# bassamlab/SigmaRL

Measured on AMD Instinct MI355X. Metric: env-steps/sec (agents x envs x steps), CPM scenario, 16 agents (open loop, 32 steps per launch), higher is better.
Workload: dtype f32

## Files before the change

sigmarl_amd/csrc/sigmaenv.hip:

```cpp
#include <hip/hip_runtime.h>

#include <algorithm>
#include <atomic>
#include <cmath>
#include <cstdio>
#include <cstdlib>
#include <cstring>
#include <string>
#include <type_traits>
#include <vector>

#include "sigmaenv_device.h"

using namespace sigmadev;

#ifdef SIGMAENV_PROFILE
#define PROF_TS2(g, tid, k) do { if ((g).dbg_ts2 && (tid) == 0) (g).dbg_ts2[(size_t)blockIdx.x * 16 + (k)] = __builtin_readcyclecounter(); } while (0)
#else
#define PROF_TS2(g, tid, k) do { } while (0)
#endif

#include "../../include/sigmaenv_ref_weights.h"
static_assert(NS >= 1 && NS <= SIGMAENV_MAX_SHORT_TERM, "SIGMAENV_N_SHORT_TERM out of range");
__device__ __constant__ uint32_t W_REF_BITS[NS] = SIGMAENV_W_REF_BITS;

#define AUTO_RESET_MAX_TRIES 64

#define DIST_STRIDE(N) ((N) + 1)
#define COL_STRIDE(N) ((N) + 4)
#define ESCR_BYTES (8 * 4 * 4 * 16)
#define CAND_LIST 16
#define ITEM_CAP(S) ((S) * 24 > 64 ? (S) * 24 : 64)
#define NEAR_CAP 8
struct Smem {
  float *st, *vold, *vnew, *shrt, *dref, *dleft, *dright, *dbound, *dist, *obs, *thr, *cs, *rew;
  float* carry;
  int *path, *cp, *near, *flags, *npts;
  unsigned long long* cmask;
  uint8_t* cand;
  uint16_t* pidx;
  float4* escr;
  uint8_t* col;
  uint16_t* items;
  unsigned long long* acc64;
  uint32_t* acc32;
  int* nearn;
  uint8_t* nearl;
  uint8_t* fresh;
  unsigned long long* key64;
  __host__ __device__ static __forceinline__ size_t scan_scratch_ints(int S) {
    return (size_t)S * 3 * 2 + (size_t)S * 2 * 4 + (size_t)S * 2 + (size_t)(ITEM_CAP(S) + 1) / 2 + (size_t)(S * 2 * NEAR_CAP + 3) / 4;
  }
  __host__ __device__ static __forceinline__ size_t stage_floats(int S, int D, bool lean) {
    const size_t o = ((size_t)S * D + 3) & ~(size_t)3, q = (scan_scratch_ints(S) + 3) & ~(size_t)3;
    return (lean && q > o) ? q : o;
  }
  __device__ __forceinline__ Smem(char* base, int S, int N, int K, int D, bool lean = false) {
    escr = reinterpret_cast<float4*>(base);
    float* f = reinterpret_cast<float*>(base + (lean ? 0 : ESCR_BYTES));
    obs = f;
    {
      int* q = reinterpret_cast<int*>(f);
      acc64 = reinterpret_cast<unsigned long long*>(q); q += S * 3 * 2;
      acc32 = reinterpret_cast<uint32_t*>(q); q += S * 2 * 4;
      nearn = q; q += S * 2;
      items = reinterpret_cast<uint16_t*>(q); q += (ITEM_CAP(S) + 1) / 2;
      nearl = reinterpret_cast<uint8_t*>(q);
    }
    f += stage_floats(S, D, lean);
    st = f; f += S * 8;
    vold = f; f += S * 10;
    vnew = f; f += S * 10;
    shrt = f; f += S * NS * 2;
    dref = f; f += S;
    dleft = f; f += S * 5;
    dright = f; f += S * 5;
    dbound = f; f += S;
    dist = f; f += S * DIST_STRIDE(N);
    thr = f; f += S * 3;
    cs = f; f += S * 2;
    rew = f; f += S * 2;
    carry = f; f += S * 3;
    int* i = reinterpret_cast<int*>(f);
    path = i; i += S;
    cp = i; i += S * 3;
    near = i; i += S * (K > 0 ? K : 1);
    flags = i; i += S * 4;
    npts = i; i += S * 3;
    i += ((reinterpret_cast<uintptr_t>(i) >> 2) & 1);
    cmask = reinterpret_cast<unsigned long long*>(i);
    if (!lean) i += S * 3 * 2;
    key64 = lean ? reinterpret_cast<unsigned long long*>(i) : cmask;
    if (lean) i += S * 2;
    cand = reinterpret_cast<uint8_t*>(i);
    if (!lean) i += S * 3 * (CAND_LIST / 4);
    pidx = reinterpret_cast<uint16_t*>(i); i += (N * (N - 1) / 2 + 1) / 2;
    col = reinterpret_cast<uint8_t*>(i);
    fresh = col + (size_t)S * COL_STRIDE(N);
  }
  __host__ __device__ static __forceinline__ size_t bytes(int S, int N, int K, int D, bool lean = false) {
    size_t f = stage_floats(S, D, lean) + (size_t)S * 8 + S * 10 * 2 + S * NS * 2 + S + S * 5 * 2 + S + (size_t)S * DIST_STRIDE(N) + S * 3 + S * 2 + S * 2 + S * 3;
    size_t i = (size_t)S + S * 3 + S * (K > 0 ? K : 1) + S * 4 + S * 3 + 1;
    i += lean ? (size_t)S * 2 : ((size_t)S * 3 * 2 + (size_t)S * 3 * (CAND_LIST / 4));
    return (lean ? 0 : ESCR_BYTES) + (f + i + (size_t)(N * (N - 1) / 2 + 1) / 2) * 4 + (size_t)S * COL_STRIDE(N) + (((size_t)S + 3) & ~(size_t)3) + 16;
  }
};

__device__ __forceinline__ void wave_sync() {
  __builtin_amdgcn_fence(__ATOMIC_RELEASE, "wavefront");
  __builtin_amdgcn_wave_barrier();
  __builtin_amdgcn_fence(__ATOMIC_ACQUIRE, "wavefront");
}
template <bool WAVE>
struct Grp {
  __device__ static __forceinline__ int tid() {
    if (!WAVE) return (int)threadIdx.x;
    int x = (int)(threadIdx.x & 63);
    asm volatile("" : "+v"(x));
    __builtin_assume(x >= 0 && x < 64);
    return x;
  }
  __device__ static __forceinline__ int size() { return WAVE ? 64 : (int)blockDim.x; }
  __device__ static __forceinline__ void sync() { if (WAVE) wave_sync(); else __syncthreads(); }
};

struct ObsLayout {
  int F, bird, full, p_steer, p_short, p_dcen, p_bnd, n_bnd_pts, own_w, oth_w, q_vel, q_steer, q_dist, q_ref, n_oth_pts, T1, pad, D, DL;
  int W_oth;
  enum { F_VERT, F_POS, F_ROT, F_LEN, F_WID, F_VEL, F_STEER, F_DIST, F_REF };
  __host__ __device__ __forceinline__ bool feature(int idx, int N, int& kind, int& wid) const {
    int n = 0;
#define SIGMA_FEAT(cond, k_, w_) if (cond) { if (idx == n) { kind = (k_); wid = (w_); return true; } ++n; }
    const bool nv = (F & SIGMAENV_OBS_NO_VERTICES) != 0;
    SIGMA_FEAT(!nv, F_VERT, 8)
    SIGMA_FEAT(nv, F_POS, 2) SIGMA_FEAT(nv, F_ROT, 1) SIGMA_FEAT(nv, F_LEN, 1) SIGMA_FEAT(nv, F_WID, 1)
    SIGMA_FEAT(true, F_VEL, 2)
    SIGMA_FEAT((F & SIGMAENV_OBS_STEERING) != 0, F_STEER, 1)
    SIGMA_FEAT(!(F & SIGMAENV_OBS_NO_DIST_AGENTS), F_DIST, N)
    SIGMA_FEAT((F & SIGMAENV_OBS_REF_OTHERS) != 0, F_REF, 2 * NS)
#undef SIGMA_FEAT
    return false;
  }
  __host__ __device__ __forceinline__ ObsLayout(int F_, int N, int K) {
    F = F_;
    bird = (F & SIGMAENV_OBS_BIRD_VIEW) != 0;
    full = (F & SIGMAENV_OBS_FULL) != 0;
    int p = bird ? 5 : 1;
    p_steer = (F & SIGMAENV_OBS_STEERING) ? p++ : -1;
    p_short = p; p += 2 * NS;
    p_dcen = (F & SIGMAENV_OBS_NO_DIST_CENTER) ? -1 : p++;
// ... 2248 lines not shown
```

sigmarl_amd/csrc/sigmaenv_step_wave.inc:

```

__device__ __forceinline__ float dpp_swap1(float v) {
  return __int_as_float(__builtin_amdgcn_update_dpp(0, __float_as_int(v), 0xB1, 0xF, 0xF, true));
}

__device__ __forceinline__ void bicycle_step_pair(const sigmaenv_config_t& c, const CfgDerived& dv, float s[8], float u0, float u1, float uc[2], float cs_yaw[2], bool par, int h, float cr[3]) {
  const float a0 = clampf(u0, -c.max_speed, c.max_speed);
  const float a1 = clampf(u1, -c.max_steering, c.max_steering);
  uc[0] = a0;
  uc[1] = a1;
  float x = s[0], y = s[1], psi = s[2], v = s[3], delta = s[4];
  float u_acc = (a0 - v) / c.dt;
  float u_sr = (a1 - delta) / c.dt;
  u_acc = clampf(u_acc, c.min_acc, c.max_acc);
  u_sr = clampf(u_sr, c.min_steering_rate, c.max_steering_rate);
  const float l_wb = dv.l_wb, k_beta = dv.k_beta;
  const float dt = c.dt;
  float delta_new = delta + dt * u_sr;
  delta_new = remainder_pos(delta_new + PI32, TWO_PI32) - PI32;
  float tan_d, beta, beta1, tan_new;
  {
    const float x1 = (par && h) ? delta_new : delta;
    const float t1 = cr_tan(x1);
    const float b1 = cr_atan(k_beta * t1);
    if (par) {
// ... 49 lines not shown
      c1 = ca;
      cr_sincos(psi, sy, cy);
    }
  }
  s[0] = x; s[1] = y; s[2] = psi; s[3] = v; s[4] = delta_new;
  s[5] = v * c1;
  s[6] = v * s1;
  s[7] = beta1;
  cs_yaw[0] = cy;
  cs_yaw[1] = sy;
  cr[0] = tan_new; cr[1] = c1; cr[2] = s1;
}

__device__ __forceinline__ void bicycle_step_pair_carried(const sigmaenv_config_t& c, const CfgDerived& dv, float s[8], float u0, float u1, float uc[2], float cs_yaw[2], int h, float cr[3]) {
  const float a0 = clampf(u0, -c.max_speed, c.max_speed);
  const float a1 = clampf(u1, -c.max_steering, c.max_steering);
  uc[0] = a0;
  uc[1] = a1;
  float x = s[0], y = s[1], psi = s[2], v = s[3], delta = s[4];
  const float beta = s[7];
  float u_acc = (a0 - v) / c.dt;
  float u_sr = (a1 - delta) / c.dt;
  u_acc = clampf(u_acc, c.min_acc, c.max_acc);
  u_sr = clampf(u_sr, c.min_steering_rate, c.max_steering_rate);
  const float l_wb = dv.l_wb, k_beta = dv.k_beta;
  const float dt = c.dt;
  float delta_new = delta + dt * u_sr;
  delta_new = remainder_pos(delta_new + PI32, TWO_PI32) - PI32;
  double sd, cd;
  sigma_sincos_f64((double)(h ? delta_new : beta), &sd, &cd);
  const float t1 = (float)(sd / cd);
  const float b1 = cr_atan(k_beta * t1);
  const float cb = (float)cd;
  const float t1o = dpp_swap1(t1), b1o = dpp_swap1(b1), cbo = dpp_swap1(cb);
  const float tan_new = h ? t1 : t1o, beta1 = h ? b1 : b1o, cosb = h ? cbo : cb;
  const float tan_d = cr[0], c0 = cr[1], s0 = cr[2];
  const float dx0 = v * c0;
  const float dx1 = v * s0;
  const float dx2 = (v / l_wb) * tan_d * cosb;
  x = x + dt * dx0;
  y = y + dt * dx1;
  psi = psi + dt * dx2;
  v = v + dt * u_acc;
  const float course = psi + beta1;
  float sa, ca;
  cr_sincos(h ? psi : course, sa, ca);
  const float so = dpp_swap1(sa), co = dpp_swap1(ca);
  const float s1 = h ? so : sa, c1 = h ? co : ca, sy = h ? sa : so, cy = h ? ca : co;
  s[0] = x; s[1] = y; s[2] = psi; s[3] = v; s[4] = delta_new;
  s[5] = v * c1;
  s[6] = v * s1;
  s[7] = beta1;
  cs_yaw[0] = cy;
  cs_yaw[1] = sy;
  cr[0] = tan_new; cr[1] = c1; cr[2] = s1;
}

__device__ __forceinline__ void rect_vertices_cs(const CfgDerived& dv, float px, float py, float cs, float sn, float* v ) {
  const float lh = dv.lh, wh = dv.wh;
  const float nsn = -sn;
  const float bx[5] = {lh, lh, -lh, -lh, lh};
  const float by[5] = {wh, -wh, -wh, wh, wh};
#pragma unroll
  for (int k = 0; k < 5; ++k) {
    v[2 * k] = (cs * bx[k] + nsn * by[k]) + px;
    v[2 * k + 1] = (sn * bx[k] + cs * by[k]) + py;
  }
}

__device__ __forceinline__ int wave_inclusive_sum(int v, int ) {
  v += __builtin_amdgcn_update_dpp(0, v, 0x111, 0xF, 0xF, false);
  v += __builtin_amdgcn_update_dpp(0, v, 0x112, 0xF, 0xF, false);
  v += __builtin_amdgcn_update_dpp(0, v, 0x114, 0xF, 0xF, false);
  v += __builtin_amdgcn_update_dpp(0, v, 0x118, 0xF, 0xF, false);
  v += __builtin_amdgcn_update_dpp(0, v, 0x142, 0xA, 0xF, false);
  v += __builtin_amdgcn_update_dpp(0, v, 0x143, 0xC, 0xF, false);
  return v;
}

struct ScanItemOut {
  float best;
  int bk;
  float bs0, bs1, bs2, bs3;
};

template <bool FASTDIV, int SEGS>
__device__ __forceinline__ void scan_chunk(const DevMap& m, const Smem& s, int sl, int pl, unsigned poly_off, int npt, int ch, int u0, bool first_of_env,
                                           const float near_thr, ScanItemOut& o) {
  const float cgx = s.st[sl * 8], cgy = s.st[sl * 8 + 1];
  const unsigned kmax = (unsigned)(npt - 2 < 0 ? 0 : npt - 2);
  Seg4 sg[SEGS];
#pragma unroll
  for (int u = 0; u < SEGS; ++u) {
    const unsigned k = min((unsigned)(ch * SIGMAENV_CHUNK + u0 + u), kmax);
    sg[u] = *reinterpret_cast<const Seg4*>(m.center + (poly_off + 2u * k));
  }
  const float* qv = first_of_env ? (s.vold + sl * 10) : (s.vnew + sl * 10);
  float q0x = 0.f, q0y = 0.f, q1x = 0.f, q1y = 0.f, q2x = 0.f, q2y = 0.f, q3x = 0.f, q3y = 0.f;
  if (pl != 0) { q0x = qv[0]; q0y = qv[1]; q1x = qv[2]; q1y = qv[3]; q2x = qv[4]; q2y = qv[5]; q3x = qv[6]; q3y = qv[7]; }
  o.bs0 = INFINITY; o.bs1 = INFINITY; o.bs2 = INFINITY; o.bs3 = INFINITY;
  unsigned near_bits = 0u;
  const float near_thr_up = __uint_as_float(__float_as_uint(near_thr) + 1u);
  float zc[SEGS];
  float zbest = INFINITY;
#pragma unroll
  for (int u = 0; u < SEGS; ++u) {
    const int k = ch * SIGMAENV_CHUNK + u0 + u;
    const bool valid = k + 1 < npt;
    const float ax = sg[u].ax, ay = sg[u].ay;
    const float lx = sg[u].bx - ax, ly = sg[u].by - ay;
    const float len2 = lx * lx + ly * ly;
    const float rcp = FASTDIV ? shared_rcp(len2) : 0.0f;
    const float z0 = point_segment_sq_t<FASTDIV>(cgx, cgy, ax, ay, lx, ly, len2, rcp);
    zc[u] = z0;
    if (valid && z0 < zbest) zbest = z0;
    if (pl != 0) {
      const float v0 = point_segment_sq_t<FASTDIV>(q0x, q0y, ax, ay, lx, ly, len2, rcp);
      const float v1 = point_segment_sq_t<FASTDIV>(q1x, q1y, ax, ay, lx, ly, len2, rcp);
      const float v2 = point_segment_sq_t<FASTDIV>(q2x, q2y, ax, ay, lx, ly, len2, rcp);
      const float v3 = point_segment_sq_t<FASTDIV>(q3x, q3y, ax, ay, lx, ly, len2, rcp);
      if (valid) {
        o.bs0 = fmin_nc(o.bs0, v0); o.bs1 = fmin_nc(o.bs1, v1); o.bs2 = fmin_nc(o.bs2, v2); o.bs3 = fmin_nc(o.bs3, v3);
        if (!(fmaf(-near_thr_up, near_thr, z0) > 0.0f)) near_bits |= 1u << u;
      }
    }
  }
  {
    const float d = sqrtf(zbest);
    const float d_up = __uint_as_float(__float_as_uint(d) + 1u);
    o.best = d; o.bk = 0x7FFFFFFF;
#pragma unroll
    for (int u = SEGS - 1; u >= 0; --u) {
      const int k = ch * SIGMAENV_CHUNK + u0 + u;
      if (k + 1 < npt && fmaf(-d_up, d, zc[u]) <= 0.0f) o.bk = k;
    }
  }
  if (near_bits) {
    const int bt = sl * 2 + (pl - 1);
    int slot = atomicAdd(&s.nearn[bt], (int)__popc(near_bits));
#pragma unroll
    for (int u = 0; u < SEGS; ++u) {
      if ((near_bits >> u) & 1u) {
        if (slot < NEAR_CAP) s.nearl[bt * NEAR_CAP + slot] = (uint8_t)(ch * SIGMAENV_CHUNK + u0 + u);
        ++slot;
      }
    }
  }
}
__device__ __forceinline__ void scan_merge(const Smem& s, int sl, int pl, const ScanItemOut& o) {
  if (o.bk != 0x7FFFFFFF) {
    const unsigned long long key = ((unsigned long long)__float_as_uint(o.best) << 32) | (unsigned)o.bk;
    atomicMin(&s.acc64[sl * 3 + pl], key);
  }
  if (pl != 0) {
    uint32_t* a = s.acc32 + (sl * 2 + (pl - 1)) * 4;
    atomicMin(&a[0], __float_as_uint(o.bs0)); atomicMin(&a[1], __float_as_uint(o.bs1));
    atomicMin(&a[2], __float_as_uint(o.bs2)); atomicMin(&a[3], __float_as_uint(o.bs3));
  }
}

template <bool FASTDIV>
__device__ __forceinline__ void scan_tile_balanced(const DevMap& m, const CfgDerived& dv, const DevBufs& g, const Smem& s, const Tile& t, int G, int lane) {
  const int N = t.N, slots = t.slots, SG = G * N, n_tasks = SG * 3, cap = ITEM_CAP(SG);
  const float near_thr = m.rect_radius + 1e-4f;
  for (int base = 0; base < n_tasks; base += 64) {
    const int tl = base + lane;
    const int grp_raw = fdiv(tl, g.mSG), sl_raw = tl - grp_raw * SG;
    const int pl_raw = grp_raw >= 2 ? 0 : grp_raw + 1;
    const int tpm = pl_raw * SG + sl_raw;
    const bool act = tl < n_tasks && sl_raw < slots;
    const int pl = act ? pl_raw : 0, sl = act ? sl_raw : 0;
    const int task = sl * 3 + pl;
    unsigned long long mk = 0ull;
#ifdef SIGMAENV_PROFILE
    int lvl_prof = 0;
#endif
    if (act) {
      MaskTask mt;
      mask_stage1(m, mt, task, s.path[sl], s.cp[task]);
      mask_stage2<true>(m, s, mt, true, N);
#ifdef SIGMAENV_PROFILE
      lvl_prof = mt.lvl;
#endif
      const float px = mt.px, py = mt.py, T2 = mt.T2;
      const int nch = mt.nch;
      unsigned long long rest = mt.rest;
      if (mt.fast && mt.own < nch) { mk |= 1ull << mt.own; rest &= ~(1ull << mt.own); }
      while (rest) {
        int idx[8];
#pragma unroll
        for (int q = 0; q < 8; ++q) { idx[q] = rest ? (__ffsll((long long)rest) - 1) : -1; rest &= rest - 1ull; }
        float4 b[8];
#pragma unroll
        for (int q = 0; q < 8; ++q) b[q] = mt.box[idx[q] < 0 ? 0 : idx[q]];
#pragma unroll
        for (int q = 0; q < 8; ++q) {
          if (idx[q] >= 0 && idx[q] < nch && box_within(b[q], px, py, T2)) mk |= 1ull << idx[q];
        }
      }
      if (!mt.fast) {
        const float4* gbox = m.group_box + ((size_t)mt.path * 3 + pl) * 8;
        unsigned gm = 0u;
#pragma unroll 1
        for (int gidx = 0; gidx < 8; ++gidx) {
          if (gidx * 8 < nch && box_within(gbox[gidx], px, py, T2)) gm |= 1u << gidx;
        }
        while (gm) {
          const int gidx = __ffs((int)gm) - 1;
          gm &= gm - 1u;
#pragma unroll 1
          for (int q = 0; q < 8; ++q) {
            const int cidx = gidx * 8 + q;
            if (cidx < nch && box_within(mt.box[cidx], px, py, T2)) mk |= 1ull << cidx;
          }
        }
      }
      s.npts[task] = mt.npt;
      s.acc64[task] = ~0ull;
      if (pl != 0) {
        const int bt = sl * 2 + (pl - 1);
        uint32_t* a = s.acc32 + bt * 4;
        a[0] = 0x7F800000u; a[1] = 0x7F800000u; a[2] = 0x7F800000u; a[3] = 0x7F800000u;
        s.nearn[bt] = 0;
      }
    }
#ifdef SIGMAENV_PROFILE
    if (g.dbg_ts && lane == 0 && base == 0) g.dbg_ts[(size_t)t.env0 / (size_t)G * 16 + 10] = __builtin_readcyclecounter();
    {
      const unsigned long long bfar = __ballot(act && lvl_prof >= 2), btight = __ballot(act && lvl_prof == 0);
#ifndef SIGMAENV_PROFILE_RT
      if (g.dbg_ts && lane == 0) {
        unsigned long long* row = g.dbg_ts + (size_t)t.env0 / (size_t)G * 16;
        row[12] += (unsigned long long)__popcll(bfar); row[13] += bfar ? 1ull : 0ull; row[14] += (unsigned long long)__popcll(btight);
        row[15] += (unsigned long long)__popcll(bfar & 0x0000000100010001ull);
      }
#endif
    }
#endif
    bool pending = act;
    do {
      const int cnt = pending ? __popcll(mk) : 0;
      const int incl = wave_inclusive_sum(cnt, lane);
      const int off = incl - cnt;
      const bool listed = pending && off + cnt <= cap;
      if (listed) {
        int j = off;
        while (mk) {
          const int ch = __ffsll((long long)mk) - 1;
          mk &= mk - 1ull;
          s.items[j++] = (uint16_t)((tpm << 6) | ch);
        }
      }
      const unsigned long long unl = __ballot(pending && !listed);
      const int total = unl ? __builtin_amdgcn_readlane(off, __builtin_amdgcn_readfirstlane(__ffsll((long long)unl) - 1)) : __builtin_amdgcn_readlane(incl, 63);
      pending = pending && !listed;
      wave_sync();
#ifdef SIGMAENV_PROFILE
      if (g.dbg_ts && lane == 0) {
        g.dbg_ts[(size_t)t.env0 / (size_t)G * 16 + 8] += (unsigned long long)total;
        g.dbg_ts[(size_t)t.env0 / (size_t)G * 16 + 9] += 1ull;
      }
#endif
      auto item_part = [&](int it, auto segs_tag, int u0) {
        constexpr int SEGS = decltype(segs_tag)::value;
        const unsigned code = s.items[it];
        const int tpm2 = (int)(code >> 6), ch = (int)(code & 63u);
        const int pl2 = fdiv(tpm2, g.mSG), sl2 = tpm2 - pl2 * SG;
        const bool first = (sl2 - fdiv(sl2, g.mN) * N) == 0;
        ScanItemOut o;
        const unsigned poly_off = (unsigned)pl2 * (unsigned)m.poly_stride + (unsigned)s.path[sl2] * (unsigned)(m.P * 2);
        scan_chunk<FASTDIV, SEGS>(m, s, sl2, pl2, poly_off, s.npts[sl2 * 3 + pl2], ch, u0, first, near_thr, o);
        scan_merge(s, sl2, pl2, o);
      };
      int it0 = 0;
      for (; it0 + 64 <= total; it0 += 64) item_part(it0 + lane, std::integral_constant<int, SIGMAENV_CHUNK>{}, 0);
      const int rem = total - it0;
      if (rem > 32) {
        if (lane < rem) item_part(it0 + lane, std::integral_constant<int, SIGMAENV_CHUNK>{}, 0);
      } else if (rem > 16) {
        if ((lane >> 1) < rem) item_part(it0 + (lane >> 1), std::integral_constant<int, SIGMAENV_CHUNK / 2>{}, (lane & 1) * (SIGMAENV_CHUNK / 2));
      } else if (rem > 0) {
        if ((lane >> 2) < rem) item_part(it0 + (lane >> 2), std::integral_constant<int, SIGMAENV_CHUNK / 4>{}, (lane & 3) * (SIGMAENV_CHUNK / 4));
      }
      wave_sync();
    } while (__any(pending));
  }
#ifdef SIGMAENV_PROFILE
  if (g.dbg_ts && lane == 0) g.dbg_ts[(size_t)t.env0 / (size_t)G * 16 + 11] = __builtin_readcyclecounter();
#endif
  const float wh = dv.wh;
  for (int tpm = lane; tpm < n_tasks; tpm += 64) {
    const int pl = fdiv(tpm, g.mSG), sl = tpm - pl * SG;
    if (sl >= slots) continue;
    const unsigned long long key = s.acc64[sl * 3 + pl];
    const float best = __uint_as_float((uint32_t)(key >> 32));
    const int bk = (int)(uint32_t)key;
    s.cp[sl * 3 + pl] = bk + 1;
    if (pl == 0) {
      s.dref[sl] = best;
    } else {
      float* dst = (pl == 1 ? s.dleft : s.dright) + sl * 5;
      dst[0] = best - wh;
    }
  }
  for (int w = lane; w < slots * 8; w += 64) {
    const int bt = w >> 2, q = w & 3, sl = bt >> 1;
    float* dst = ((bt & 1) ? s.dright : s.dleft) + sl * 5;
    dst[1 + q] = sqrtf(__uint_as_float(s.acc32[w]));
  }
}

template <int SN>
struct PairTable {
  uint16_t v[SN * (SN - 1) / 2 > 0 ? SN * (SN - 1) / 2 : 1];
  constexpr PairTable() : v() {
    int k = 0;
    for (int i = 0; i < SN - 1; ++i)
      for (int j = i + 1; j < SN; ++j) v[k++] = (uint16_t)(i | (j << 8));
  }
};
template <int SN>
__device__ const PairTable<SN> kPairTable{};

#ifndef STEP_WAVE_MIN_WAVES
#define STEP_WAVE_MIN_WAVES 4
#endif
struct StepKernArgs {
  DevMap m;
  DevBufs g;
  const float* actions_base;
  float* slab_base;
  size_t act_stride, slab_stride;
  uint64_t seed, counter0;
  int G_arg, tile_lds, path_first, path_count, n_steps;
};
template <class T>
__device__ __forceinline__ T* as_global(T* p) {
  return (T*)(__attribute__((address_space(1))) T*)p;
}
#define SIGMA_COPY_GLOBAL(dst, src, f) dst.f = as_global(src.f)
__device__ __forceinline__ void load_step_tables(const __attribute__((address_space(4))) StepKernArgs* ka, DevMap& m, DevBufs& g) {
  SIGMA_COPY_GLOBAL(m, ka->m, center); SIGMA_COPY_GLOBAL(m, ka->m, left); SIGMA_COPY_GLOBAL(m, ka->m, right); SIGMA_COPY_GLOBAL(m, ka->m, yaw);
  SIGMA_COPY_GLOBAL(m, ka->m, n_center); SIGMA_COPY_GLOBAL(m, ka->m, n_left); SIGMA_COPY_GLOBAL(m, ka->m, n_right); SIGMA_COPY_GLOBAL(m, ka->m, is_loop);
  SIGMA_COPY_GLOBAL(m, ka->m, chunk_box); SIGMA_COPY_GLOBAL(m, ka->m, group_box); SIGMA_COPY_GLOBAL(m, ka->m, chunk_neigh); SIGMA_COPY_GLOBAL(m, ka->m, start_table);
  m.P = ka->m.P; m.n_paths = ka->m.n_paths; m.yaw_stride = ka->m.yaw_stride; m.neigh_radius = ka->m.neigh_radius; m.neigh_radius_far = ka->m.neigh_radius_far;
  m.nch = ka->m.nch; m.fast_div = ka->m.fast_div; m.rect_radius = ka->m.rect_radius; m.poly_stride = ka->m.poly_stride;
  m.n_lists = ka->m.n_lists; m.neigh_radius_tight = ka->m.neigh_radius_tight;
  m.list_first16 = ka->m.list_first16; m.list_count16 = ka->m.list_count16; m.cdf0 = ka->m.cdf0; m.cdf1 = ka->m.cdf1; m.cdf2 = ka->m.cdf2;
  SIGMA_COPY_GLOBAL(g, ka->g, state); SIGMA_COPY_GLOBAL(g, ka->g, prev_pos); SIGMA_COPY_GLOBAL(g, ka->g, vertices); SIGMA_COPY_GLOBAL(g, ka->g, short_term);
  SIGMA_COPY_GLOBAL(g, ka->g, dist_ref); SIGMA_COPY_GLOBAL(g, ka->g, dist_left); SIGMA_COPY_GLOBAL(g, ka->g, dist_right); SIGMA_COPY_GLOBAL(g, ka->g, dist_bound);
  SIGMA_COPY_GLOBAL(g, ka->g, dist_agents); SIGMA_COPY_GLOBAL(g, ka->g, reward); SIGMA_COPY_GLOBAL(g, ka->g, reward_info); SIGMA_COPY_GLOBAL(g, ka->g, obs);
  SIGMA_COPY_GLOBAL(g, ka->g, action); SIGMA_COPY_GLOBAL(g, ka->g, cbf_nominal); SIGMA_COPY_GLOBAL(g, ka->g, path); SIGMA_COPY_GLOBAL(g, ka->g, closest);
  SIGMA_COPY_GLOBAL(g, ka->g, nearing); SIGMA_COPY_GLOBAL(g, ka->g, timer); SIGMA_COPY_GLOBAL(g, ka->g, col_agents); SIGMA_COPY_GLOBAL(g, ka->g, col_flags);
  SIGMA_COPY_GLOBAL(g, ka->g, done); SIGMA_COPY_GLOBAL(g, ka->g, reset_mask); SIGMA_COPY_GLOBAL(g, ka->g, reset_full); SIGMA_COPY_GLOBAL(g, ka->g, fresh);
  SIGMA_COPY_GLOBAL(g, ka->g, slab); SIGMA_COPY_GLOBAL(g, ka->g, dbg_ts2); SIGMA_COPY_GLOBAL(g, ka->g, dbg_ts);
  SIGMA_COPY_GLOBAL(g, ka->g, lanelet_centers); SIGMA_COPY_GLOBAL(g, ka->g, lanelet_neigh); SIGMA_COPY_GLOBAL(g, ka->g, bnd_left);
  SIGMA_COPY_GLOBAL(g, ka->g, bnd_n_center); SIGMA_COPY_GLOBAL(g, ka->g, bnd_is_loop);
  g.n_lanelets = ka->g.n_lanelets; g.lanelet_pts = ka->g.lanelet_pts; g.bnd_poly_stride = ka->g.bnd_poly_stride; g.bnd_P = ka->g.bnd_P; g.mVT1 = ka->g.mVT1;
  g.obs_salt = 0u;
  g.mN = ka->g.mN; g.mT1 = ka->g.mT1; g.mT2 = ka->g.mT2; g.mTP = ka->g.mTP; g.mW = ka->g.mW; g.mSG = ka->g.mSG; g.dbg_skip = ka->g.dbg_skip;
}
#undef SIGMA_COPY_GLOBAL

template <bool FASTDIV, bool PAR, int SN = 0, int SG = 0, bool VAR = false, bool MTVS = false>
__global__ void __launch_bounds__(256, STEP_WAVE_MIN_WAVES) sigmaenv_step_wave_kernel(const sigmaenv_config_t* __restrict__ cfg_dev, StepKernArgs args) {
  sigma_poison_lds();
  extern __shared__ __attribute__((aligned(16))) char smem_raw[];
  const int lane0 = threadIdx.x & 63;
  {
    const int wave0 = __builtin_amdgcn_readfirstlane(threadIdx.x >> 6);
    const int tile0 = blockIdx.x * (blockDim.x >> 6) + wave0;
    if (tile0 * (SN ? SG : args.G_arg) >= cfg_dev->n_envs) return;
  }
#ifdef SIGMAENV_PROFILE
#define TSW(k) do { unsigned long long* ts_ = as_global(ka->g.dbg_ts); if (ts_ && lane == 0) ts_[(size_t)tile_index * 16 + (k)] = __builtin_readcyclecounter(); } while (0)
#define SKIP(bit) (ka->g.dbg_skip & (bit))
#else
#define TSW(k) do { } while (0)
#define SKIP(bit) false
#endif
#if defined(SIGMAENV_PROFILE) && defined(SIGMAENV_PROFILE_RT)
#define TSRT(k) do { unsigned long long* ts_ = as_global(ka->g.dbg_ts); if (ts_ && lane == 0) ts_[(size_t)tile_index * 16 + (k)] = __builtin_amdgcn_s_memrealtime(); } while (0)
#else
#define TSRT(k) do { } while (0)
#endif
  for (int step_i = 0;; ++step_i) {
  int lane = lane0;
  unsigned long long kap = (unsigned long long)__builtin_amdgcn_kernarg_segment_ptr();
  asm volatile("" : "+v"(lane));
  __builtin_assume(lane >= 0 && lane < 64);
  asm volatile("" : "+s"(kap));
  struct KernargLayout { const sigmaenv_config_t* cfg_dev; StepKernArgs a; };
  const __attribute__((address_space(4))) StepKernArgs* ka = (const __attribute__((address_space(4))) StepKernArgs*)(kap + __builtin_offsetof(KernargLayout, a));
  if (step_i >= ka->n_steps) break;
  if (ka->n_steps > 1) {
    const int pr = 3 - (step_i & 3);
    switch (pr) {
      case 3: __builtin_amdgcn_s_setprio(3); break;
      case 2: __builtin_amdgcn_s_setprio(2); break;
      case 1: __builtin_amdgcn_s_setprio(1); break;
      default: __builtin_amdgcn_s_setprio(0); break;
    }
  }
  const int wave = __builtin_amdgcn_readfirstlane((int)(threadIdx.x >> 6)), tile_index = blockIdx.x * (blockDim.x >> 6) + wave;
  const int tile_lds = ka->tile_lds;
#define STEP_KA(kav) asm volatile("" : "+s"(kap)); const __attribute__((address_space(4))) StepKernArgs* kav = (const __attribute__((address_space(4))) StepKernArgs*)(kap + __builtin_offsetof(KernargLayout, a))
#define STEP_TABLES(mv, gv)                                                                                                                 \
  DevMap mv;                                                                                                                                \
  DevBufs gv;                                                                                                                               \
  {                                                                                                                                         \
    STEP_KA(ka_);                                                                                                                           \
    load_step_tables(ka_, mv, gv);                                                                                                          \
    if (SN > 0) {                                                                                                                           \
      constexpr int SK_ = 2;                                                                                                                \
      gv.mN = magic_u32(SN); gv.mT1 = magic_u32(NS + 4 * SK_); gv.mT2 = magic_u32(SK_ + 1); gv.mTP = magic_u32(SN * (SN - 1) / 2);        \
      if (!VAR) gv.mW = magic_u32(SN * (4 + 2 * NS + 11 * SK_ + 1) + 1);                                                                  \
      gv.mSG = magic_u32((SG > 0 ? SG : 1) * SN);                                                                                         \
    }                                                                                                                                       \
  }
  int cfg_zero = 0;
  asm volatile("" : "+s"(cfg_zero));
  const sigmaenv_config_t& c = cfg_dev[cfg_zero];
  const CfgDerived& dv = reinterpret_cast<const DevConfig*>(cfg_dev)[cfg_zero].d;
  const int G = SN ? SG : ka->G_arg;
  Tile t(c, G, tile_index);
  if (SN > 0) {
    constexpr int SK = 2;
    t.N = SN; t.K = SK;
    if (!VAR) { t.D = 4 + 2 * NS + 11 * SK; t.DL = t.D; }
    if (SG == 1) { t.nenv = 1; t.env0 = tile_index; }
    t.slots = t.nenv * SN; t.a0 = (size_t)t.env0 * SN;
  }
  const int N = t.N;
  char* base = smem_raw + (size_t)wave * tile_lds;
  Smem s(base, G * N, N, t.K, t.DL, true);
  unsigned long long* s_mask = reinterpret_cast<unsigned long long*>(base + ((Smem::bytes(G * N, N, t.K, t.DL, true) + 15) & ~(size_t)15));
  int* s_full = reinterpret_cast<int*>(s_mask + G);
  int* s_any = s_full + G;
  int* s_tim = reinterpret_cast<int*>(base + ((Smem::bytes(G * N, N, t.K, t.DL, true) + 15) & ~(size_t)15) + 16 * (size_t)G + 16);
  const bool first = step_i == 0, last = step_i + 1 >= ka->n_steps;
  TSW(0);
  if (first) TSRT(12);
#if defined(SIGMAENV_PROFILE) && defined(SIGMAENV_PROFILE_RT)
  { unsigned long long* ts_ = as_global(ka->g.dbg_ts); if (ts_ && lane == 0) ts_[(size_t)tile_index * 16 + 15] = (unsigned long long)__builtin_amdgcn_s_getreg(4 | (31 << 11)) | ((unsigned long long)__builtin_amdgcn_s_getreg(20 | (31 << 11)) << 32); }
#endif
  if (SN == 0 && step_i == 0) {
    for (int i = lane; i < N - 1; i += 64) {
      const int off = i * (2 * N - i - 1) / 2;
      for (int j = i + 1; j < N; ++j) s.pidx[off + j - i - 1] = (uint16_t)(i | (j << 8));
    }
  }
  {
    STEP_TABLES(m, g);
    STEP_KA(ka_a);
    const float* __restrict__ actions = as_global(ka_a->actions_base) + (size_t)step_i * ka_a->act_stride;
    constexpr bool par = PAR;
    const int sl_raw = par ? (lane >> 1) : lane, h = par ? (lane & 1) : 0;
    const bool act = sl_raw < t.slots;
    const int sl = act ? sl_raw : 0;
    const size_t gi = t.a0 + sl;
    float st[8], uc[2], csy[2];
    const float2 u = reinterpret_cast<const float2*>(actions)[gi];
    float4 s0, s1;
    int pth, cp0, cp1, cp2;
    float2 vo[5], pp, spo[NS];
    int4 tm;
    if (first) {
      const float4* gs = reinterpret_cast<const float4*>(g.state + gi * 8);
      s0 = gs[0]; s1 = gs[1];
      pth = g.path[gi * 4];
      const float2* gv = reinterpret_cast<const float2*>(g.vertices + gi * 10);
#pragma unroll
      for (int k = 0; k < 5; ++k) vo[k] = gv[k];
      cp0 = g.closest[gi * 3 + 0]; cp1 = g.closest[gi * 3 + 1]; cp2 = g.closest[gi * 3 + 2];
      pp = reinterpret_cast<const float2*>(g.prev_pos)[gi];
      const float2* gst = reinterpret_cast<const float2*>(g.short_term + gi * NS * 2);
#pragma unroll
      for (int k = 0; k < NS; ++k) spo[k] = gst[k];
      tm = reinterpret_cast<const int4*>(g.timer)[t.env0 + fdiv(sl, g.mN)];
      if (act && h == 0 && sl - fdiv(sl, g.mN) * N == 0) s_tim[fdiv(sl, g.mN) * 4 + 3] = tm.w;
    } else {
      const float4* ls = reinterpret_cast<const float4*>(s.st + sl * 8);
      s0 = ls[0]; s1 = ls[1];
      pth = s.path[sl];
#pragma unroll
      for (int k = 0; k < 5; ++k) vo[k] = make_float2(s.vnew[sl * 10 + 2 * k], s.vnew[sl * 10 + 2 * k + 1]);
      cp0 = s.cp[sl * 3 + 0]; cp1 = s.cp[sl * 3 + 1]; cp2 = s.cp[sl * 3 + 2];
      pp = make_float2(s0.x, s0.y);
#pragma unroll
      for (int k = 0; k < NS; ++k) spo[k] = make_float2(s.shrt[sl * NS * 2 + 2 * k], s.shrt[sl * NS * 2 + 2 * k + 1]);
      tm = reinterpret_cast<const int4*>(s_tim)[fdiv(sl, g.mN)];
    }
    const int loop_flag = m.is_loop[pth];
    st[0] = s0.x; st[1] = s0.y; st[2] = s0.z; st[3] = s0.w; st[4] = s1.x; st[5] = s1.y; st[6] = s1.z; st[7] = s1.w;
    float cr3[3] = {0.f, 1.f, 0.f};
    if (par && !first) { cr3[0] = s.carry[sl * 3]; cr3[1] = s.carry[sl * 3 + 1]; cr3[2] = s.carry[sl * 3 + 2]; }
    if (SKIP(1)) { uc[0] = u.x; uc[1] = u.y; csy[0] = 1.f; csy[1] = 0.f; }
    else if (par && !first) bicycle_step_pair_carried(c, dv, st, u.x, u.y, uc, csy, h, cr3);
    else bicycle_step_pair(c, dv, st, u.x, u.y, uc, csy, par, h, cr3);
    float v[10];
    rect_vertices_cs(dv, st[0], st[1], csy[0], csy[1], v);
    if (act && h == 0) {
#pragma unroll
      for (int k = 0; k < 8; ++k) s.st[sl * 8 + k] = st[k];
      if (last) {
        reinterpret_cast<float2*>(g.action)[gi] = make_float2(uc[0], uc[1]);
        float4* go = reinterpret_cast<float4*>(g.state + gi * 8);
        go[0] = make_float4(st[0], st[1], st[2], st[3]);
        go[1] = make_float4(st[4], st[5], st[6], st[7]);
      }
      s.cs[sl * 2] = csy[0]; s.cs[sl * 2 + 1] = csy[1];
      s.carry[sl * 3] = cr3[0]; s.carry[sl * 3 + 1] = cr3[1]; s.carry[sl * 3 + 2] = cr3[2];
      s.path[sl] = pth;
      s.fresh[sl] = 0;
      s.thr[sl * 3] = pp.x; s.thr[sl * 3 + 1] = pp.y;
      s.thr[sl * 3 + 2] = __int_as_float(tm.x);
      s.flags[sl * 4 + 1] = loop_flag;
      s.flags[sl * 4 + 2] = tm.y;
      s.near[sl * (t.K > 0 ? t.K : 1)] = tm.z;
      s.cp[sl * 3 + 0] = cp0; s.cp[sl * 3 + 1] = cp1; s.cp[sl * 3 + 2] = cp2;
    }
    if (act && h == (par ? 1 : 0)) {
      float2* gvo = reinterpret_cast<float2*>(g.vertices + gi * 10);
#pragma unroll
      for (int k = 0; k < 5; ++k) {
        s.vold[sl * 10 + 2 * k] = vo[k].x; s.vold[sl * 10 + 2 * k + 1] = vo[k].y;
        s.vnew[sl * 10 + 2 * k] = v[2 * k]; s.vnew[sl * 10 + 2 * k + 1] = v[2 * k + 1];
        if (last) gvo[k] = make_float2(v[2 * k], v[2 * k + 1]);
      }
#pragma unroll
      for (int k = 0; k < NS; ++k) { s.shrt[sl * NS * 2 + 2 * k] = spo[k].x; s.shrt[sl * NS * 2 + 2 * k + 1] = spo[k].y; }
    }
  }
  wave_sync();
  TSW(1);
  {
  STEP_TABLES(m, g);
  if (SKIP(2)) {
  } else if (m.nch > 0) {
    scan_tile_balanced<FASTDIV>(m, dv, g, s, t, G, lane);
  } else {
    for (int sl = 0; sl < t.slots; ++sl) {
      const int i = sl % N;
      const float* si = s.st + sl * 8;
      const float* qv = (i == 0) ? (s.vold + sl * 10) : (s.vnew + sl * 10);
      AgentScan r;
      agent_scan_full<true>(m, c, s.path[sl], lane, si[0], si[1], qv, s.vnew + sl * 10, r);
      if (lane == 0) {
        s.dref[sl] = r.d_ref;
#pragma unroll
        for (int q = 0; q < 5; ++q) { s.dleft[sl * 5 + q] = r.dl[q]; s.dright[sl * 5 + q] = r.dr[q]; }
        s.cp[sl * 3 + 0] = r.cp_ref; s.cp[sl * 3 + 1] = r.cp_l; s.cp[sl * 3 + 2] = r.cp_r;
        s.npts[sl * 3] = m.n_center[s.path[sl]];
        s.flags[sl * 4 + 0] = r.hit ? 1 : 0;
      }
    }
  }
  }
  wave_sync();
  TSW(2);
  {
  STEP_TABLES(m, g);
  (void)g;
  if (m.nch > 0 && !SKIP(4)) {
    for (int base = 0; base < t.slots * 2; base += 16) {
      const int bt = base + (lane >> 2), e4 = lane & 3;
      const bool act = bt < t.slots * 2;
      const int btc = act ? bt : 0;
      const int sl = btc >> 1, side = btc & 1;
      const int nn = act ? s.nearn[btc] : 0;
      const float* pv = s.vnew + sl * 10 + 2 * e4;
      const Edge ed = make_edge(pv[0], pv[1], pv[2], pv[3]);
      const unsigned poly_off = (unsigned)(side + 1) * (unsigned)m.poly_stride + (unsigned)s.path[sl] * (unsigned)(m.P * 2);
      const bool all = nn > NEAR_CAP;
      const int cnt = all ? (s.npts[sl * 3 + 1 + side] - 1) : nn;
      bool hit = false;
      constexpr int PRE = 4;
      Seg4 pre[PRE];
#pragma unroll
      for (int j = 0; j < PRE; ++j) {
        const unsigned k = (j < cnt) ? (all ? (unsigned)j : (unsigned)s.nearl[btc * NEAR_CAP + (j < NEAR_CAP ? j : 0)]) : 0u;
        pre[j] = *reinterpret_cast<const Seg4*>(m.center + (poly_off + 2u * k));
      }
#pragma unroll
      for (int j = 0; j < PRE; ++j) {
        if (j < cnt) {
          const Seg4 sg = pre[j];
          const float lx = sg.bx - sg.ax, ly = sg.by - sg.ay;
          const float S2 = lx * sg.ay - ly * sg.ax;
          hit |= edge_hits_segment(ed, sg.ax, sg.ay, sg.bx, sg.by, lx, ly, S2);
        }
      }
      for (int j = PRE; __any(j < cnt); ++j) {
        if (j < cnt) {
          const unsigned k = all ? (unsigned)j : (unsigned)s.nearl[btc * NEAR_CAP + j];
          const Seg4 sg = *reinterpret_cast<const Seg4*>(m.center + (poly_off + 2u * k));
          const float lx = sg.bx - sg.ax, ly = sg.by - sg.ay;
          const float S2 = lx * sg.ay - ly * sg.ax;
          hit |= edge_hits_segment(ed, sg.ax, sg.ay, sg.bx, sg.by, lx, ly, S2);
        }
      }
      const unsigned long long hb = __ballot(hit);
      if (act && (lane & 7) == 0) s.flags[sl * 4 + 0] = ((hb >> lane) & 0xFFull) ? 1 : 0;
    }
  }
  }
  TSW(3);
  {
  STEP_TABLES(m, g);
  if (!SKIP(8)) {
    const float diag = dv.diag;
    const int TP = N * (N - 1) / 2;
    const int n_pairs = t.nenv * TP;
    const bool pen_staged = !c.is_testing_mode && (c.rew_flags & SIGMAENV_REW_DISTANCE) && N <= t.DL;
    const float pen_x0 = c.threshold_near_other_agents_low, pen_x1 = c.threshold_near_other_agents_high;
    const float pen_den = pen_x1 - pen_x0;
    const bool pen_fast = pen_den >= 0x1p-60f && pen_den <= 0x1p60f;
    const float pen_rcp = pen_fast ? shared_rcp(pen_den) : 0.0f;
    auto pen_term = [&](float d) {
      const float x = clampf(d, pen_x0, pen_x1);
      const float q = pen_fast ? div_shared(x - pen_x0, pen_den, pen_rcp) : (x - pen_x0) / pen_den;
      return 1.0f - q;
    };
    const bool mtv_staged = MTVS && c.distance_type != SIGMAENV_DIST_C2C && N + MTV_REC <= t.DL;
    float* mtv_rec = s.obs + t.slots * N;
    wave_sync();
    for (int sl = lane; sl < t.slots; sl += 64) {
      const int i = sl - fdiv(sl, g.mN) * N;
      s.dist[sl * DIST_STRIDE(N) + i] = diag;
      s.col[sl * COL_STRIDE(N) + i] = 0;
      if (pen_staged) s.obs[sl * N + i] = pen_term(diag);
    }
    if (mtv_staged) {
      for (int sl = lane; sl < t.slots; sl += 64) rect_mtv_record(s.vold + sl * 10, mtv_rec + sl * MTV_REC);
      wave_sync();
    }
    for (int base = 0; base < n_pairs; base += 64) {
      const int p = base + lane;
      const bool in_range = p < n_pairs;
      int si = 0, sj = 0, i = 0, j = 0;
      bool near = false;
      if (in_range) {
        const int e = fdiv(p, g.mTP);
        const unsigned ij = SN > 0 ? kPairTable<(SN > 0 ? SN : 2)>.v[p - e * TP] : s.pidx[p - e * TP];
        i = (int)(ij & 0xFFu); j = (int)(ij >> 8);
        si = e * N + i; sj = e * N + j;
        float d;
        if (!mtv_staged) d = pair_distance(c, s.st, s.vold, si, sj);
        else d = mtv_pair_staged(s.vold + si * 10, s.vold + sj * 10, mtv_rec + si * MTV_REC, mtv_rec + sj * MTV_REC);
        s.dist[si * DIST_STRIDE(N) + j] = d;
        s.dist[sj * DIST_STRIDE(N) + i] = d;
        if (pen_staged) { const float pt = pen_term(d); s.obs[si * N + j] = pt; s.obs[sj * N + i] = pt; }
        uint8_t col = 0;
        if (c.distance_type == SIGMAENV_DIST_C2C) {
          near = !(d > 2.0f * m.rect_radius + 1e-4f);
        } else {
          col = (d == 0.0f) ? 1 : 0;
        }
        if (!near) { s.col[si * COL_STRIDE(N) + j] = col; s.col[sj * COL_STRIDE(N) + i] = col; }
      }
      unsigned long long todo = __ballot(near);
      while (todo) {
        const int q = lane >> 4, tt = lane & 15;
        unsigned long long rest = todo;
        int src = -1;
#pragma unroll
        for (int k = 0; k < 4; ++k) {
          const int b = rest ? (__ffsll((long long)rest) - 1) : -1;
          if (k == q) src = b;
          rest &= rest - 1ull;
        }
        todo = rest;
        const int a_sl = __shfl(si, src < 0 ? 0 : src, 64), b_sl = __shfl(sj, src < 0 ? 0 : src, 64);
        bool hit = false;
        if (src >= 0) {
          const float* va = s.vnew + a_sl * 10 + 2 * (tt >> 2);
          const float* vb = s.vnew + b_sl * 10 + 2 * (tt & 3);
          const Edge ed = make_edge(va[0], va[1], va[2], va[3]);
          const float dx2 = vb[2] - vb[0], dy2 = vb[3] - vb[1];
          const float S2 = dx2 * vb[1] - dy2 * vb[0];
          hit = edge_hits_segment(ed, vb[0], vb[1], vb[2], vb[3], dx2, dy2, S2);
        }
        const unsigned long long hb = __ballot(hit);
        if (src >= 0 && tt == 0) {
          const uint8_t col = ((hb >> (q * 16)) & 0xFFFFull) ? 1 : 0;
          const int ea = fdiv(a_sl, g.mN) * N;
// ... 274 lines not shown
```

Baseline: 3.004 billion.

## Compact near-boundary segment candidates into a global list and test them flat

Near-boundary segment candidates were stored in fixed per-agent/side buckets using shared atomics. They now go into one wave-wide compacted list of 16-bit codes, with slots assigned by a DPP prefix sum. The collision test then spreads (candidate, edge) pairs evenly across lanes instead of iterating per agent with divergent loop counts. Hit flags are cleared at step start and set by direct writes, and an all-segment fallback runs when the list overflows. This removes load imbalance and per-bucket atomics, at the cost of extra prefix-sum work in the scan loop and a dependence on the shared counter.

New measurement: 3.064 billion (median of 6 runs). +2.0%, better.

```diff
diff --git a/sigmarl_amd/csrc/sigmaenv.hip b/sigmarl_amd/csrc/sigmaenv.hip
--- a/sigmarl_amd/csrc/sigmaenv.hip
+++ b/sigmarl_amd/csrc/sigmaenv.hip
@@ -45,11 +45,12 @@
   unsigned long long* acc64;
   uint32_t* acc32;
   int* nearn;
-  uint8_t* nearl;
+  uint16_t* nearl;
+  int* nearc;
   uint8_t* fresh;
   unsigned long long* key64;
   __host__ __device__ static __forceinline__ size_t scan_scratch_ints(int S) {
-    return (size_t)S * 3 * 2 + (size_t)S * 2 * 4 + (size_t)S * 2 + (size_t)(ITEM_CAP(S) + 1) / 2 + (size_t)(S * 2 * NEAR_CAP + 3) / 4;
+    return (size_t)S * 3 * 2 + (size_t)S * 2 * 4 + (size_t)S * 2 + (size_t)(ITEM_CAP(S) + 1) / 2 + (size_t)(S * NEAR_CAP + 1) / 2;
   }
   __host__ __device__ static __forceinline__ size_t stage_floats(int S, int D, bool lean) {
     const size_t o = ((size_t)S * D + 3) & ~(size_t)3, q = (scan_scratch_ints(S) + 3) & ~(size_t)3;
@@ -65,7 +66,8 @@
       acc32 = reinterpret_cast<uint32_t*>(q); q += S * 2 * 4;
       nearn = q; q += S * 2;
       items = reinterpret_cast<uint16_t*>(q); q += (ITEM_CAP(S) + 1) / 2;
-      nearl = reinterpret_cast<uint8_t*>(q);
+      nearl = reinterpret_cast<uint16_t*>(q);
+      nearc = nullptr;
     }
     f += stage_floats(S, D, lean);
     st = f; f += S * 8;
diff --git a/sigmarl_amd/csrc/sigmaenv_step_wave.inc b/sigmarl_amd/csrc/sigmaenv_step_wave.inc
--- a/sigmarl_amd/csrc/sigmaenv_step_wave.inc
+++ b/sigmarl_amd/csrc/sigmaenv_step_wave.inc
@@ -155,6 +155,7 @@
   float best;
   int bk;
   float bs0, bs1, bs2, bs3;
+  unsigned near_bits;
 };
 
 template <bool FASTDIV, int SEGS>
@@ -208,17 +209,8 @@
       if (k + 1 < npt && fmaf(-d_up, d, zc[u]) <= 0.0f) o.bk = k;
     }
   }
-  if (near_bits) {
-    const int bt = sl * 2 + (pl - 1);
-    int slot = atomicAdd(&s.nearn[bt], (int)__popc(near_bits));
-#pragma unroll
-    for (int u = 0; u < SEGS; ++u) {
-      if ((near_bits >> u) & 1u) {
-        if (slot < NEAR_CAP) s.nearl[bt * NEAR_CAP + slot] = (uint8_t)(ch * SIGMAENV_CHUNK + u0 + u);
-        ++slot;
-      }
-    }
-  }
+  o.near_bits = near_bits;
+  if (near_bits) atomicAdd(&s.nearn[sl * 2 + (pl - 1)], (int)__popc(near_bits));
 }
 __device__ __forceinline__ void scan_merge(const Smem& s, int sl, int pl, const ScanItemOut& o) {
   if (o.bk != 0x7FFFFFFF) {
@@ -234,8 +226,22 @@
 
 template <bool FASTDIV>
 __device__ __forceinline__ void scan_tile_balanced(const DevMap& m, const CfgDerived& dv, const DevBufs& g, const Smem& s, const Tile& t, int G, int lane) {
-  const int N = t.N, slots = t.slots, SG = G * N, n_tasks = SG * 3, cap = ITEM_CAP(SG);
+  const int N = t.N, slots = t.slots, SG = G * N, n_tasks = SG * 3, cap = ITEM_CAP(SG), near_cap = SG * NEAR_CAP;
   const float near_thr = m.rect_radius + 1e-4f;
+  int near_total = 0;
+  auto near_append = [&](unsigned nb, int code0) {
+    const int cnt = (int)__popc(nb);
+    const int incl = wave_inclusive_sum(cnt, lane);
+    int slot = near_total + incl - cnt;
+    near_total += __builtin_amdgcn_readlane(incl, 63);
+#pragma unroll
+    for (int u = 0; u < SIGMAENV_CHUNK; ++u) {
+      if ((nb >> u) & 1u) {
+        if (slot < near_cap) s.nearl[slot] = (uint16_t)(code0 + u);
+        ++slot;
+      }
+    }
+  };
   for (int base = 0; base < n_tasks; base += 64) {
     const int tl = base + lane;
     const int grp_raw = fdiv(tl, g.mSG), sl_raw = tl - grp_raw * SG;
@@ -334,7 +340,7 @@
         g.dbg_ts[(size_t)t.env0 / (size_t)G * 16 + 9] += 1ull;
       }
 #endif
-      auto item_part = [&](int it, auto segs_tag, int u0) {
+      auto item_part = [&](int it, auto segs_tag, int u0, unsigned& nb, int& code0) {
         constexpr int SEGS = decltype(segs_tag)::value;
         const unsigned code = s.items[it];
         const int tpm2 = (int)(code >> 6), ch = (int)(code & 63u);
@@ -344,23 +350,34 @@
         const unsigned poly_off = (unsigned)pl2 * (unsigned)m.poly_stride + (unsigned)s.path[sl2] * (unsigned)(m.P * 2);
         scan_chunk<FASTDIV, SEGS>(m, s, sl2, pl2, poly_off, s.npts[sl2 * 3 + pl2], ch, u0, first, near_thr, o);
         scan_merge(s, sl2, pl2, o);
+        nb = o.near_bits;
+        code0 = ((sl2 * 2 + (pl2 - 1)) << 8) | (ch * SIGMAENV_CHUNK + u0);
       };
       int it0 = 0;
-      for (; it0 + 64 <= total; it0 += 64) item_part(it0 + lane, std::integral_constant<int, SIGMAENV_CHUNK>{}, 0);
+      for (; it0 + 64 <= total; it0 += 64) {
+        unsigned nb = 0u;
+        int code0 = 0;
+        item_part(it0 + lane, std::integral_constant<int, SIGMAENV_CHUNK>{}, 0, nb, code0);
+        near_append(nb, code0);
+      }
       const int rem = total - it0;
+      unsigned nb = 0u;
+      int code0 = 0;
       if (rem > 32) {
-        if (lane < rem) item_part(it0 + lane, std::integral_constant<int, SIGMAENV_CHUNK>{}, 0);
+        if (lane < rem) item_part(it0 + lane, std::integral_constant<int, SIGMAENV_CHUNK>{}, 0, nb, code0);
       } else if (rem > 16) {
-        if ((lane >> 1) < rem) item_part(it0 + (lane >> 1), std::integral_constant<int, SIGMAENV_CHUNK / 2>{}, (lane & 1) * (SIGMAENV_CHUNK / 2));
+        if ((lane >> 1) < rem) item_part(it0 + (lane >> 1), std::integral_constant<int, SIGMAENV_CHUNK / 2>{}, (lane & 1) * (SIGMAENV_CHUNK / 2), nb, code0);
       } else if (rem > 0) {
-        if ((lane >> 2) < rem) item_part(it0 + (lane >> 2), std::integral_constant<int, SIGMAENV_CHUNK / 4>{}, (lane & 3) * (SIGMAENV_CHUNK / 4));
-      }
+        if ((lane >> 2) < rem) item_part(it0 + (lane >> 2), std::integral_constant<int, SIGMAENV_CHUNK / 4>{}, (lane & 3) * (SIGMAENV_CHUNK / 4), nb, code0);
+      }
+      if (rem > 0) near_append(nb, code0);
       wave_sync();
     } while (__any(pending));
   }
 #ifdef SIGMAENV_PROFILE
   if (g.dbg_ts && lane == 0) g.dbg_ts[(size_t)t.env0 / (size_t)G * 16 + 11] = __builtin_readcyclecounter();
 #endif
+  if (lane == 0) *s.nearc = near_total;
   const float wh = dv.wh;
   for (int tpm = lane; tpm < n_tasks; tpm += 64) {
     const int pl = fdiv(tpm, g.mSG), sl = tpm - pl * SG;
@@ -510,6 +527,7 @@
   unsigned long long* s_mask = reinterpret_cast<unsigned long long*>(base + ((Smem::bytes(G * N, N, t.K, t.DL, true) + 15) & ~(size_t)15));
   int* s_full = reinterpret_cast<int*>(s_mask + G);
   int* s_any = s_full + G;
+  s.nearc = s_any + 1;
   int* s_tim = reinterpret_cast<int*>(base + ((Smem::bytes(G * N, N, t.K, t.DL, true) + 15) & ~(size_t)15) + 16 * (size_t)G + 16);
   const bool first = step_i == 0, last = step_i + 1 >= ka->n_steps;
   TSW(0);
@@ -588,6 +606,7 @@
       s.fresh[sl] = 0;
       s.thr[sl * 3] = pp.x; s.thr[sl * 3 + 1] = pp.y;
       s.thr[sl * 3 + 2] = __int_as_float(tm.x);
+      s.flags[sl * 4 + 0] = 0;
       s.flags[sl * 4 + 1] = loop_flag;
       s.flags[sl * 4 + 2] = tm.y;
       s.near[sl * (t.K > 0 ? t.K : 1)] = tm.z;
@@ -635,46 +654,51 @@
   {
   STEP_TABLES(m, g);
   (void)g;
-  if (m.nch > 0 && !SKIP(4)) {
-    for (int base = 0; base < t.slots * 2; base += 16) {
-      const int bt = base + (lane >> 2), e4 = lane & 3;
-      const bool act = bt < t.slots * 2;
-      const int btc = act ? bt : 0;
-      const int sl = btc >> 1, side = btc & 1;
-      const int nn = act ? s.nearn[btc] : 0;
-      const float* pv = s.vnew + sl * 10 + 2 * e4;
-      const Edge ed = make_edge(pv[0], pv[1], pv[2], pv[3]);
-      const unsigned poly_off = (unsigned)(side + 1) * (unsigned)m.poly_stride + (unsigned)s.path[sl] * (unsigned)(m.P * 2);
-      const bool all = nn > NEAR_CAP;
-      const int cnt = all ? (s.npts[sl * 3 + 1 + side] - 1) : nn;
-      bool hit = false;
-      constexpr int PRE = 4;
-      Seg4 pre[PRE];
-#pragma unroll
-      for (int j = 0; j < PRE; ++j) {
-        const unsigned k = (j < cnt) ? (all ? (unsigned)j : (unsigned)s.nearl[btc * NEAR_CAP + (j < NEAR_CAP ? j : 0)]) : 0u;
-        pre[j] = *reinterpret_cast<const Seg4*>(m.center + (poly_off + 2u * k));
-      }
-#pragma unroll
-      for (int j = 0; j < PRE; ++j) {
-        if (j < cnt) {
-          const Seg4 sg = pre[j];
+  if (m.nch > 0 && !SKIP(4) && !SKIP(2)) {
+    const int total = __builtin_amdgcn_readfirstlane(*s.nearc), near_cap = G * N * NEAR_CAP;
+#ifdef SIGMAENV_PROFILE
+    if (g.dbg_ts && lane == 0) {
+      g.dbg_ts[(size_t)tile_index * 16 + 8] += (unsigned long long)total << 32;
+      g.dbg_ts[(size_t)tile_index * 16 + 9] += (unsigned long long)(total > near_cap ? 1 : 0) << 32;
+    }
+#endif
+    if (total <= near_cap) {
+      const int n_tests = total * 4, e4 = lane & 3;
+      for (int base = 0; base < n_tests; base += 64) {
+        const int w = base + lane;
+        const unsigned code = s.nearl[min(w, n_tests - 1) >> 2];
+        const int bt = (int)(code >> 8), sl = bt >> 1, side = bt & 1;
+        const unsigned poly_off = (unsigned)(side + 1) * (unsigned)m.poly_stride + (unsigned)s.path[sl] * (unsigned)(m.P * 2);
+        const Seg4 sg = *reinterpret_cast<const Seg4*>(m.center + (poly_off + 2u * (code & 255u)));
+        if (w < n_tests) {
+          const float* pv = s.vnew + sl * 10 + 2 * e4;
+          const Edge ed = make_edge(pv[0], pv[1], pv[2], pv[3]);
           const float lx = sg.bx - sg.ax, ly = sg.by - sg.ay;
           const float S2 = lx * sg.ay - ly * sg.ax;
-          hit |= edge_hits_segment(ed, sg.ax, sg.ay, sg.bx, sg.by, lx, ly, S2);
-        }
-      }
-      for (int j = PRE; __any(j < cnt); ++j) {
-        if (j < cnt) {
-          const unsigned k = all ? (unsigned)j : (unsigned)s.nearl[btc * NEAR_CAP + j];
-          const Seg4 sg = *reinterpret_cast<const Seg4*>(m.center + (poly_off + 2u * k));
-          const float lx = sg.bx - sg.ax, ly = sg.by - sg.ay;
-          const float S2 = lx * sg.ay - ly * sg.ax;
-          hit |= edge_hits_segment(ed, sg.ax, sg.ay, sg.bx, sg.by, lx, ly, S2);
-        }
-      }
-      const unsigned long long hb = __ballot(hit);
-      if (act && (lane & 7) == 0) s.flags[sl * 4 + 0] = ((hb >> lane) & 0xFFull) ? 1 : 0;
+          if (edge_hits_segment(ed, sg.ax, sg.ay, sg.bx, sg.by, lx, ly, S2)) s.flags[sl * 4 + 0] = 1;
+        }
+      }
+    } else {
+      for (int base = 0; base < t.slots * 2; base += 16) {
+        const int bt = base + (lane >> 2), e4 = lane & 3;
+        const bool act = bt < t.slots * 2;
+        const int btc = act ? bt : 0;
+        const int sl = btc >> 1, side = btc & 1;
+        const int cnt = (act && s.nearn[btc] > 0) ? (s.npts[sl * 3 + 1 + side] - 1) : 0;
+        const float* pv = s.vnew + sl * 10 + 2 * e4;
+        const Edge ed = make_edge(pv[0], pv[1], pv[2], pv[3]);
+        const unsigned poly_off = (unsigned)(side + 1) * (unsigned)m.poly_stride + (unsigned)s.path[sl] * (unsigned)(m.P * 2);
+        bool hit = false;
+        for (int j = 0; __any(j < cnt); ++j) {
+          if (j < cnt) {
+            const Seg4 sg = *reinterpret_cast<const Seg4*>(m.center + (poly_off + 2u * (unsigned)j));
+            const float lx = sg.bx - sg.ax, ly = sg.by - sg.ay;
+            const float S2 = lx * sg.ay - ly * sg.ax;
+            hit |= edge_hits_segment(ed, sg.ax, sg.ay, sg.bx, sg.by, lx, ly, S2);
+          }
+        }
+        if (hit) s.flags[sl * 4 + 0] = 1;
+      }
     }
   }
   }
```
